# Samsung/iac

Measured on AMD Instinct MI355X. Metric: Msamples/s rendered (3rd-order HOA->binaural, 48 kHz), higher is better.
Workload: dtype f32

## Files before the change

### iac_amd/__init__.py

```python
from .hipabi import (
    FMT_F32,
    FMT_S16,
    FMT_S24,
    FMT_S32,
    KIND_DMX,
    KIND_FIR,
    KIND_H2M,
    KIND_M2M,
    PROJ_AUTO,
    PROJ_EXACT,
    PROJ_MFMA,
    SS,
    Batch,
    BatchConfig,
    DemixConfig,
    DemixFrame,
    DemixState,
    DmxFrame,
    DmxState,
    FANOUT_MAX,
    RenderArgs,
    Resampler,
    dmx_matrix,
    fir_matrix,
    IamfHipError,
    LpcmLayout,
    LpcmInput,
    Matrix,
    build,
    get_h2m_matrix,
    get_m2m_matrix,
    layout_channels,
    lib,
    lib_path,
    lpcm_unpack,
    render_fanout,
    ROUTE,
    RouteRow,
    route_instances,
    route_reset,
    route_tally,
)
```

### iac_amd/csrc/iamf_render.hip

```cpp
#include <hip/hip_runtime.h>

#include <math.h>
#include <stdint.h>
#include <atomic>
#include <stdio.h>
#include <stdlib.h>
#include <string.h>

#include <new>
#include <type_traits>
#include <vector>

#include "../../include/iamf_hip.h"

#define IAMF_FFT_HOST_TABLES

#include "render_entry.hpp"

namespace {

#include "render_common.hpp"
#include "render_downmix.hpp"
#include "render_fir.hpp"
#include "render_fir16.hpp"
// ... 72 lines not shown
  static Tables t(false), t_tv(true);
  return tv ? t_tv : t;
}

int find_matrix(int kind, int in_id, int out_id, iamf_hip_matrix *out, bool tv = false) {
  const Tables &t = tables(tv);
  if (!t.ok || !out) return -1;
  for (int i = 0; i < t.n; ++i) {
    const TableEntry &e = t.ents[i];
    if ((int)e.kind == kind && (int)e.in_id == in_id && (int)e.out_id == out_id) {
      out->kind = kind;
      out->in_id = in_id;
      out->out_id = out_id;
      out->channels = e.channels;
      out->lfe1 = e.lfe1;
      out->lfe2 = e.lfe2;
      out->m = e.m;
      out->n = e.n;
      out->mat = t.data + e.offset;
      return 0;
    }
  }
  return -1;
}

float ease(float x) {
  if (1.0 < x) return 1.0f;
  if (x < 0) return 0.0f;
  return 1.0f - powf(x - 1, 2.0);
}

}

struct iamf_hip_batch {
  iamf_hip_batch_config cfg;
  int device = 0;
  hipEvent_t done = nullptr;
  bool rendered = false;
  int m = 0, n_feeds = 0;
  int32_t src_feed[kMaxOut];
  uint32_t nz_mask[6] = {0, 0, 0, 0, 0, 0};
  int sparse = 0;
  int32_t *d_src_feed = nullptr;
  float thr = 0.f;
  int n_atk = 0, n_end = 0;
  std::vector<int64_t> spos;
  std::vector<uint8_t> sflushed;
  bool any_rendered = false;
  bool lp_scale_ok = false;
  float *d_matrix = nullptr, *d_gains = nullptr, *d_ctab = nullptr, *d_ring_y = nullptr,
        *d_ring_pm = nullptr;
  LimState *d_lim = nullptr;
  std::vector<float> h_gains;
  bool has2 = false;
  int m2 = 0;
  float *d_matrix2 = nullptr, *d_gains2 = nullptr;
  int32_t *d_src_feed2 = nullptr, *d_dmx_tab = nullptr;
  bool dmx = false;
  int dmx_n_in = 0, dmx_n_out = 0;
  float *d_pre = nullptr;
  int pre_l = 0;
  std::vector<float> h_fm;
  float *d_matrix_pre = nullptr;
  uint32_t nz_mask_pre[6] = {0, 0, 0, 0, 0, 0};
  int sparse_pre = 0;
  bool demix = false;
  int demix_steps = 0, demix_skip = 0, demix_layout = 0, demix_gmask = 0, demix_w4 = 0;
  int32_t *d_demix_tab = nullptr;
  float *d_demix_ftab = nullptr;
  bool fir = false;
  int fir_taps = 0;
  float *d_fir_hist[2] = {nullptr, nullptr};
  void *d_fir_h16 = nullptr;
  float *d_fir_pq = nullptr, *d_fir_tw = nullptr;
  float *d_fir_zero = nullptr;
  float *d_fir_pre[2] = {nullptr, nullptr};
  size_t fir_pre_bytes = 0;
  float *d_fir_y = nullptr;
  size_t fir_y_floats = 0;
  float *d_lp_in = nullptr;
  size_t lp_in_floats = 0;
  float *d_fir_id = nullptr;
  int32_t *d_fir_id_feed = nullptr;
  float fir_inv_scale = 1.f;
  int fir_cur = 0;
  bool lfe = false;
  float lfe_a1 = 0.f, lfe_a2 = 0.f, lfe_a3 = 0.f, lfe_b1 = 0.f, lfe_b2 = 0.f;
  double lfe_div = 0.0;
  float *d_lfe_state = nullptr, *d_lfe_next = nullptr, *d_lfe_u = nullptr;
  bool lfe_shared = false;
  size_t lfe_u_floats = 0;
  uint8_t *d_nat = nullptr;
  size_t nat_bytes = 0;
  uint8_t *d_dump = nullptr;
};

namespace {

bool on_batch_device(const iamf_hip_batch *b) {
  int dev = -1;
  return hipGetDevice(&dev) == hipSuccess && dev == b->device;
}

int quiesce(iamf_hip_batch *b) {
  if (b->rendered) HIPCHK(hipEventSynchronize(b->done));
  return IAMF_HIP_OK;
// ... 521 lines not shown
    b->dmx_n_out = mx.n;
    for (int i = 0; i < mx.m; ++i) dmx_tab[i] = kLayoutCh[mx.in_id][i];
    for (int i = 0; i < mx.n; ++i) dmx_tab[12 + i] = kLayoutCh[mx.out_id][i];
  } else if (fir) {
    for (int i = 0; i < kMaxOut; ++i) b->src_feed[i] = -1;
    fm.assign(mx.mat, mx.mat + (size_t)2 * mx.m * cfg->fir_taps);
  } else {
    build_feed_map(mx, cfg->out_channels, fm, b->src_feed);
    b->lp_scale_ok = true;
    for (float w : fm)
      if (w != 0.f && !(fabsf(w) >= 0x1p-100f && fabsf(w) <= 0x1p100f)) b->lp_scale_ok = false;
    if (cfg->lfe_hoa && mx.kind == IAMF_HIP_KIND_H2M && (mx.lfe1 >= 0 || mx.lfe2 >= 0)) {
      const float sample_rate = (float)cfg->sample_rate, cutoff_freq = 120;
      const float delta_time = 1 / sample_rate + 1.0e-10;
      const float c = 1.0f / (float)tanf(M_PI * cutoff_freq * delta_time);
      b->lfe = true;
      b->lfe_a1 = 1.0f / (1.0f + c + c * c);
      b->lfe_a2 = 2.0f * b->lfe_a1;
      b->lfe_a3 = b->lfe_a1;
      b->lfe_b1 = 2.0f * (1.0f - c * c) * b->lfe_a1;
      b->lfe_b2 = (1.0f - c + c * c) * b->lfe_a1;
      b->lfe_div = mx.n <= 2 ? 0.0 : sqrt((double)mx.n);
      if (mx.lfe1 >= 0 && mx.lfe1 < cfg->out_channels) b->src_feed[mx.lfe1] = -2;
      if (mx.lfe2 >= 0 && mx.lfe2 < cfg->out_channels) b->src_feed[mx.lfe2] = -2;
    }
    int set = 0, all = 0;
    for (int g = 0; g < 6 && 4 * g < cfg->out_channels; ++g)
      for (int k = 0; k < mx.m && k < 32; ++k) {
        bool nz = false;
        for (int c = 4 * g; c < 4 * g + 4 && c < cfg->out_channels; ++c)
          if (b->src_feed[c] >= 0 && fm[(size_t)b->src_feed[c] * mx.m + k] != 0.f) nz = true;
        ++all;
        if (nz) {
          ++set;
          b->nz_mask[g] |= 1u << k;
        }
      }
    b->sparse = 2 * set < all ? 1 : 0;
    b->h_fm = fm;
  }

  const float atk = 0.001f, rel = 0.200f;
  b->thr = (float)pow(10, cfg->limiter_threshold_db / 20);
  const float inc = (float)1 / (float)cfg->sample_rate;
  std::vector<float> T;
  T.push_back(0.0f);
  while (T.back() < rel + atk && T.size() < (1u << 22)) T.push_back(T.back() + inc);
  b->n_end = (int)T.size() - 1;
  b->n_atk = 0;
  while (b->n_atk < b->n_end && T[b->n_atk] < atk) ++b->n_atk;
  std::vector<float> ctab((size_t)b->n_end + 1, 1.0f);
  for (int k = 1; k <= b->n_end; ++k)
    ctab[k] = (k - 1) < b->n_atk ? ease(T[k] / atk) : ease((T[k] - atk) / rel);

  const int ns = cfg->n_streams;
  b->h_gains.assign((size_t)3 * ns, 1.0f);
#define CREATE_CHK(expr)                       \
  do {                                         \
    if ((expr) != hipSuccess) {                \
      iamf_hip_batch_destroy(b);               \
      return IAMF_HIP_ERR_DEVICE;              \
    }                                          \
  } while (0)
  CREATE_CHK(hipEventCreateWithFlags(&b->done, hipEventDisableTiming));
  CREATE_CHK(hipMalloc(&b->d_matrix, sizeof(float) * fm.size()));
  CREATE_CHK(hipMalloc(&b->d_gains, sizeof(float) * 3 * ns));
  CREATE_CHK(hipMalloc(&b->d_ctab, sizeof(float) * ctab.size()));
  CREATE_CHK(hipMalloc(&b->d_lim, sizeof(LimState) * ns));
  CREATE_CHK(hipMalloc(&b->d_ring_y, sizeof(float) * (size_t)ns * cfg->out_channels * kSave));
  CREATE_CHK(hipMalloc(&b->d_ring_pm, sizeof(float) * (size_t)ns * kSave));
  if (b->lfe) {
    CREATE_CHK(hipMalloc(&b->d_lfe_state, sizeof(float) * 4 * (size_t)ns));
    CREATE_CHK(hipMalloc(&b->d_lfe_next, sizeof(float) * 2 * (size_t)ns));
  }
  CREATE_CHK(hipMalloc(&b->d_dump, (size_t)ns * 256 * 16));
  CREATE_CHK(hipMalloc(&b->d_src_feed, sizeof(int32_t) * kMaxOut));
  CREATE_CHK(hipMemcpy(b->d_src_feed, b->src_feed, sizeof(int32_t) * kMaxOut, hipMemcpyHostToDevice));
  if (fir) {
    const size_t hb = sizeof(float) * (size_t)ns * mx.m * 256;
    CREATE_CHK(hipMalloc(&b->d_fir_hist[0], hb));
    CREATE_CHK(hipMalloc(&b->d_fir_hist[1], hb));
    CREATE_CHK(hipMemset(b->d_fir_hist[0], 0, hb));
    CREATE_CHK(hipMemset(b->d_fir_hist[1], 0, hb));
    const int taps = cfg->fir_taps;
    float hmax = 0.f;
    for (size_t i = 0; i < (size_t)2 * mx.m * taps; ++i) hmax = fmaxf(hmax, fabsf(mx.mat[i]));
    if (hmax > 0.f && hmax < 1e30f) {
      int e = 0;
      (void)frexpf(hmax, &e);
      const float scale = ldexpf(1.f, 14 - e);
      std::vector<_Float16> tab((size_t)mx.m * 2 * 2 * 8 * kF16Taps, (_Float16)0.f);
      for (int ch = 0; ch < mx.m; ++ch)
        for (int ear = 0; ear < 2; ++ear)
          for (int r = 0; r < 8; ++r)
            for (int n = 0; n < kF16Taps; ++n) {
              const int k = n + r - 15;
              if (k < 0 || k >= taps) continue;
              const float v = mx.mat[((size_t)ear * mx.m + ch) * taps + k] * scale;
              const _Float16 hi = (_Float16)v;
              const _Float16 lo = (_Float16)((v - (float)hi) * 2048.f);
              const size_t at = ((((size_t)ch * 2 + ear) * 2 + 0) * 8 + r) * kF16Taps + n;
              tab[at] = hi;
              tab[at + (size_t)8 * kF16Taps] = lo;
            }
      CREATE_CHK(hipMalloc(&b->d_fir_h16, tab.size() * sizeof(_Float16)));
      CREATE_CHK(hipMemcpy(b->d_fir_h16, tab.data(), tab.size() * sizeof(_Float16), hipMemcpyHostToDevice));
// ... 196 lines not shown
  hipStream_t st = static_cast<hipStream_t>(args->stream);
  const size_t need = (size_t)ns * nf * ch * fs;
  if (need > b->lp_in_floats) {
    const int q = quiesce(b);
    if (q != IAMF_HIP_OK) return q;
    HIPCHK(hipStreamSynchronize(st));
    (void)hipFree(b->d_lp_in);
    b->d_lp_in = nullptr;
    b->lp_in_floats = 0;
    HIPCHK(hipMalloc(&b->d_lp_in, sizeof(float) * need));
    HIPCHK(hipMemset(b->d_lp_in, 0, sizeof(float) * need));
    b->lp_in_floats = need;
  }
  const int fmax = 65535 / n_streams > 0 ? 65535 / n_streams : 0;
  if (fmax == 0) return IAMF_HIP_ERR_UNIMPLEMENTED;
  const int64_t lp_stream_stride = (int64_t)nf * ch * fs;
  for (int f = 0; f < nf; f += fmax) {
    const int r = iamf_hip_lpcm_unpack_frames(
        &L, static_cast<const uint8_t *>(in->d_raw) + (int64_t)stream0 * in->raw_stream_stride + (int64_t)f * in->raw_frame_stride,
        in->raw_stream_stride, in->raw_frame_stride, nf - f < fmax ? nf - f : fmax, nullptr, 0,
        b->d_lp_in + (int64_t)stream0 * lp_stream_stride + (size_t)f * ch * fs, lp_stream_stride, (int64_t)ch * fs, n_streams, st, first,
        count);
    if (r != IAMF_HIP_OK) return r;
  }
  a.d_in = b->d_lp_in;
  a.in_stream_stride = lp_stream_stride;
  a.in_frame_stride = (int64_t)ch * fs;
  return render_range_impl(b, &a, stream0, n_streams, nullptr);
}

int iamf_hip_batch_render_ex(iamf_hip_batch *b, const iamf_hip_render_args *a) {
  if (!b) return IAMF_HIP_ERR_BAD_ARG;
  return iamf_hip_batch_render_range(b, a, 0, b->cfg.n_streams);
}

int iamf_hip_batch_render(iamf_hip_batch *b, const float *d_in, int64_t in_stream_stride,
                          int64_t in_frame_stride, int32_t n_frames, void *d_pcm,
                          int64_t pcm_stream_stride_bytes, void *stream) {
  iamf_hip_render_args a;
  memset(&a, 0, sizeof(a));
  a.d_in = d_in;
  a.in_stream_stride = in_stream_stride;
  a.in_frame_stride = in_frame_stride;
  a.n_frames = n_frames;
  a.d_pcm = d_pcm;
  a.pcm_stream_stride_bytes = pcm_stream_stride_bytes;
  a.stream = stream;
  if (b && (b->has2 || b->dmx || b->demix)) return IAMF_HIP_ERR_BAD_ARG;
  return iamf_hip_batch_render_ex(b, &a);
}

static const int kFanFuseMax = IAMF_HIP_FANOUT_MAX;

int iamf_hip_batch_render_fanout(iamf_hip_batch *const *batches, int32_t n_batches, const float *d_in, int64_t in_stream_stride,
                                 int64_t in_frame_stride, int32_t n_frames, void *const *d_pcm,
                                 const int64_t *pcm_stream_stride_bytes, void *stream, int32_t *n_emitted, int32_t *n_fused) {
  if (n_batches < 1 || n_batches > IAMF_HIP_FANOUT_MAX) return IAMF_HIP_ERR_BAD_ARG;
  if (!batches || !d_in || !d_pcm || !pcm_stream_stride_bytes || !n_emitted) return IAMF_HIP_ERR_BAD_ARG;
  for (int j = 0; j < n_batches; ++j) {
    if (!batches[j] || !d_pcm[j]) return IAMF_HIP_ERR_BAD_ARG;
    for (int i = 0; i < j; ++i)
      if (batches[i] == batches[j]) return IAMF_HIP_ERR_BAD_ARG;
  }
  iamf_hip_render_args args[IAMF_HIP_FANOUT_MAX];
  int64_t total = 0;
  const iamf_hip_batch *b0 = batches[0];
  for (int j = 0; j < n_batches; ++j) {
    const iamf_hip_batch *b = batches[j];
    if (b->cfg.n_streams != b0->cfg.n_streams || b->cfg.frame_size != b0->cfg.frame_size || b->m != b0->m ||
        (b->d_pre ? b->pre_l : b->m) != (b0->d_pre ? b0->pre_l : b0->m))
      return IAMF_HIP_ERR_BAD_ARG;
    if (b->has2 || b->dmx || b->demix) return IAMF_HIP_ERR_BAD_ARG;
    iamf_hip_render_args &a = args[j];
    memset(&a, 0, sizeof(a));
    a.d_in = d_in;
    a.in_stream_stride = in_stream_stride;
    a.in_frame_stride = in_frame_stride;
    a.n_frames = n_frames;
    a.d_pcm = d_pcm[j];
    a.pcm_stream_stride_bytes = pcm_stream_stride_bytes[j];
    a.stream = stream;
    int64_t tj = 0;
    const int rc = range_args_check(b, &a, 0, b->cfg.n_streams, &tj);
    if (rc != IAMF_HIP_OK) return rc;
    total = tj;
  }
  if (total == 0) {
    if (n_fused) *n_fused = 0;
    for (int j = 0; j < n_batches; ++j) n_emitted[j] = 0;
    return IAMF_HIP_OK;
  }
  for (int j = 0; j < n_batches; ++j) {
    const iamf_hip_batch *b = batches[j];
    if (!on_batch_device(b)) return IAMF_HIP_ERR_INVALID_STATE;
    for (int i = 0; i < b->cfg.n_streams; ++i)
      if (b->spos[(size_t)i] != b0->spos[0] || b->sflushed[(size_t)i]) return IAMF_HIP_ERR_INVALID_STATE;
  }
  if (n_fused) *n_fused = 0;
  for (int j = 0; j < n_batches; ++j) n_emitted[j] = 0;

  const int ns = b0->cfg.n_streams;
  PreparedCall pcs[IAMF_HIP_FANOUT_MAX];
  bool fuse[IAMF_HIP_FANOUT_MAX];
  int k = 0;
  for (int j = 0; j < n_batches; ++j) {
    iamf_hip_batch *b = batches[j];
    fuse[j] = false;
    const int sc = b->cfg.pcm_stride_channels;
    if (k >= kFanFuseMax || b->fir || b->lfe || b->d_pre || (sc > 0 && sc != b->cfg.out_channels) || !b->cfg.limiter_enable ||
        b->cfg.out_channels > 2)
      continue;
    const int rc = render_prepare(b, args[j], (int)total, 0, ns, nullptr, pcs[j]);
    if (rc != IAMF_HIP_OK) return rc;
    const Route r = pick_route(pcs[j].p, pcs[j].m_eff);
    fuse[j] = r.family == Family::Fast && r.variant == 0 && pcs[j].m_eff == b0->m && FanM::has(pcs[j].m_eff);
    if (fuse[j]) ++k;
  }
  if (k < 2) k = 0;
  if (k) {
    FanParams fp;
    memset(&fp, 0, sizeof(fp));
    int n = 0;
    for (int j = 0; j < n_batches; ++j) {
      if (!fuse[j]) continue;
      const RenderParams &p = pcs[j].p;
      if (n == 0) {
        fp.in = p.in;
        fp.in_stream_stride = p.in_stream_stride;
        fp.in_frame_stride = p.in_frame_stride;
        fp.pos0 = p.pos0;
        fp.total = p.total;
        fp.frame_size = p.frame_size;
        fp.n_streams = p.n_streams;
        fp.stream0 = 0;
        fp.n_launch = ns;
      }
      FanMember &mb = fp.mem[n++];
      mb.pcm = p.pcm;
      mb.pcm_stream_stride = p.pcm_stream_stride;
      mb.matrix = p.matrix;
      mb.gains = p.gains;
      mb.ctab = p.ctab;
      mb.lim = p.lim;
      mb.ring_y = p.ring_y;
      mb.ring_pm = p.ring_pm;
      mb.src_feed = p.src_feed;
      mb.out_ch = p.out_ch;
      mb.out_format = p.out_format;
      mb.loudness_on = p.loudness_on;
      mb.n_atk = p.n_atk;
      mb.n_end = p.n_end;
      mb.thr = p.thr;
    }
    if (!iamf_hip_fanout_launch(&fp, b0->m, k, static_cast<hipStream_t>(stream))) return IAMF_HIP_ERR_INTERNAL;
    HIPCHK(hipGetLastError());
    iamf_hip_route_count(IAMF_HIP_ROUTE_FANOUT, 0, b0->m, 0, k);
    for (int j = 0; j < n_batches; ++j) {
      if (!fuse[j]) continue;
      const int r = render_commit(batches[j], pcs[j]);
      if (r < 0) return r;
      n_emitted[j] = r;
    }
    if (n_fused) *n_fused = k;
  }
  for (int j = 0; j < n_batches; ++j) {
    if (k && fuse[j]) continue;
    const int r = render_call(batches[j], args[j], (int)total, 0, ns);
    if (r < 0) return r;
    n_emitted[j] = r;
  }
  return IAMF_HIP_OK;
}

int iamf_hip_batch_flush_range(iamf_hip_batch *b, void *d_pcm, int64_t pcm_stream_stride_bytes, void *stream,
                               int32_t stream0, int32_t n_streams) {
  if (!b || !d_pcm) return IAMF_HIP_ERR_BAD_ARG;
  if (stream0 < 0 || n_streams <= 0 || stream0 + n_streams > b->cfg.n_streams) return IAMF_HIP_ERR_BAD_ARG;
  for (int i = stream0; i < stream0 + n_streams; ++i)
    if (b->sflushed[(size_t)i]) return IAMF_HIP_ERR_INVALID_STATE;
  if (!b->cfg.limiter_enable) return 0;
  iamf_hip_render_args a;
  memset(&a, 0, sizeof(a));
  a.d_pcm = d_pcm;
  a.pcm_stream_stride_bytes = pcm_stream_stride_bytes;
  a.stream = stream;
  const int r = render_call(b, a, kDelay, stream0, n_streams);
  if (r >= 0)
    for (int i = stream0; i < stream0 + n_streams; ++i) b->sflushed[(size_t)i] = 1;
  return r;
}

int iamf_hip_batch_flush(iamf_hip_batch *b, void *d_pcm, int64_t pcm_stream_stride_bytes, void *stream) {
  if (!b) return IAMF_HIP_ERR_BAD_ARG;
  return iamf_hip_batch_flush_range(b, d_pcm, pcm_stream_stride_bytes, stream, 0, b->cfg.n_streams);
}

int iamf_hip_batch_set_second_element(iamf_hip_batch *b, const iamf_hip_matrix *mx, const float *g2) {
  if (b && !on_batch_device(b)) return IAMF_HIP_ERR_INVALID_STATE;
  if (!b || !mx || !mx->mat || mx->m <= 0 || mx->m > kMaxIn || mx->n <= 0 || mx->n > kMaxOut ||
      mx->kind == IAMF_HIP_KIND_DMX || b->any_rendered)
    return IAMF_HIP_ERR_BAD_ARG;
  std::vector<float> fm;
  int32_t feed[kMaxOut];
  build_feed_map(*mx, b->cfg.out_channels, fm, feed);
  const int ns = b->cfg.n_streams;
  std::vector<float> gains((size_t)ns, 1.0f);
  if (g2) memcpy(gains.data(), g2, sizeof(float) * ns);
  (void)hipFree(b->d_matrix2);
  (void)hipFree(b->d_gains2);
// ... 298 lines not shown
```

### iac_amd/csrc/iamf_render_fanout.hip

```cpp
#include <hip/hip_runtime.h>

#include <stdint.h>
#include <atomic>
#include <stdlib.h>
#include <string.h>

#include <type_traits>

#include "../../include/iamf_hip.h"
#include "render_entry.hpp"

namespace {

#include "render_common.hpp"
#include "render_downmix.hpp"
#include "render_fir.hpp"
#include "render_fir16.hpp"
#include "render_fir_fft.hpp"
#include "render_fast.hpp"
#include "render_fanout.hpp"

static_assert(2 * sizeof(float) * fan_lds_floats(3, 16) <= 160 * 1024, "K = 2 and 3: two workgroups per CU");
static_assert(sizeof(float) * fan_lds_floats(kFanMax, 16) <= 160 * 1024, "K = 4 fits a CU");

static_assert(FanK::has(2) && FanK::has(kFanMax) && !FanK::has(kFanMax + 1), "FanK is 2..kFanMax");

template <int M, int K>
void launch_fan_mk(const FanParams &p, hipStream_t st) {
  constexpr size_t lds = sizeof(float) * (size_t)fan_lds_floats(K, M);
  launch_big_lds<&render_fanout_kernel<M, K>, (int)lds>(dim3((unsigned)p.n_launch), dim3(256), lds, st, p);
}

}

int iamf_hip_fanout_launch(const void *params, int m, int k, hipStream_t st) {
  FanParams p;
  memcpy(&p, params, sizeof(p));
  for (int j = 0; j < k && j < kFanMax; ++j)
    if (p.mem[j].out_ch < 1 || p.mem[j].out_ch > 2) return 0;
  return dispatch(FanM{}, m, [&](auto M) {
    return dispatch(FanK{}, k, [&](auto K) { launch_fan_mk<M.value, K.value>(p, st); });
  });
}
```

### iac_amd/csrc/render_fanout.hpp

```cpp
#pragma once

constexpr int kFanMax = IAMF_HIP_FANOUT_MAX;

struct FanMember {
  uint8_t *pcm;
  int64_t pcm_stream_stride;
  const float *matrix;
  const float *gains;
  const float *ctab;
  LimState *lim;
  float *ring_y;
  float *ring_pm;
  const int32_t *src_feed;
  int32_t out_ch;
  int32_t out_format;
  int32_t loudness_on;
  int32_t n_atk, n_end;
  float thr;
};

struct FanParams {
  const float *in;
  int64_t in_stream_stride;
  int64_t in_frame_stride;
  int64_t pos0;
  int32_t total;
  int32_t frame_size;
  int32_t n_streams;
  int32_t stream0, n_launch;
  FanMember mem[kFanMax];
};

__host__ __device__ constexpr int fan_member_floats() { return 3 * kFRing + 2 * (kFRing / 16) + kSave + 2 * kFWin; }
__host__ __device__ constexpr int fan_lds_floats(int k, int m) {
  return k * fan_member_floats() + kFChunk + ((2 * k * m + 15) & ~15) + 16;
}

template <int M, int K>
__global__ __launch_bounds__(256, K <= 3 ? 2 : 1) void render_fanout_kernel(const FanParams p) {
  static_assert(K >= 2 && K <= kFanMax, "two to four members");
  extern __shared__ float lds[];
  constexpr int R = kFRing;
  constexpr int NB = R / 16;
  constexpr int MB = fan_member_floats();
  constexpr int NS = 2 * K;
  constexpr int oSuf = 2 * R, oBm = 3 * R, oPm = 3 * R + 2 * NB, oWin = oPm + kSave, oHead = oWin + kFWin;
  float *arr_p = lds + K * MB;
  float *arr_g = arr_p;
  float *mat = arr_p + kFChunk;
  float *misc = mat + ((NS * M + 15) & ~15);
  constexpr bool kWG = (M % 4) == 0;

  const int s = blockIdx.x + p.stream0;
  const int t = (int)threadIdx.x;
  const int wave = t >> 6;
  const int lane = t & 63;
  const int q = t & 3;
  const int fs = p.frame_size;
  int base = (int)((p.pos0 & ~(int64_t)15) % R);

  float g_cur[K], gs[K], ge[K], m_eg[K], m_og[K], m_lg[K];
  int n_st[K];
  bool any_gain[K], live[K][2];
#pragma unroll
  for (int j = 0; j < K; ++j) {
    const FanMember &mb = p.mem[j];
    float *my = lds + j * MB;
    const int oc = mb.out_ch;
    const float *sy = mb.ring_y + (int64_t)s * oc * kSave;
    const float *spm = mb.ring_pm + (int64_t)s * kSave;
    const int rp = ring_wrap(base - kSave + t);
#pragma unroll
    for (int c = 0; c < 2; ++c)
      if (c < oc) my[c * R + rp] = sy[c * kSave + t];
    const float pm = spm[t];
    my[oPm + t] = pm;
    float sfx = pm;
    sfx = fmaxf(sfx, __shfl_down(sfx, 1, 16));
    sfx = fmaxf(sfx, __shfl_down(sfx, 2, 16));
    sfx = fmaxf(sfx, __shfl_down(sfx, 4, 16));
    sfx = fmaxf(sfx, __shfl_down(sfx, 8, 16));
    my[oSuf + rp] = sfx;
    if ((t & 15) == 0) my[oBm + (rp >> 4)] = my[oBm + (rp >> 4) + NB] = sfx;
    const int n_end = mb.n_end;
    for (int i = t; i < kFWin; i += 256) my[oHead + i] = mb.ctab[i < n_end ? i : n_end];
    if (t < 2 * M) {
      const int c = t / M, m = t - c * M;
      const int f = c < oc ? mb.src_feed[c] : -1;
      mat[2 * j * M + t] = f >= 0 ? mb.matrix[f * M + m] : 0.f;
    }
    const LimState ls = mb.lim[s];
    g_cur[j] = ls.g, gs[j] = ls.gs, ge[j] = ls.ge, n_st[j] = ls.n;
    const float eg = mb.gains[s], og = mb.gains[p.n_streams + s], lg = mb.gains[2 * p.n_streams + s];
    const bool eg_on = (eg != 1.f && eg > 0.f);
    const bool og_on = (og != 1.f && og > 0.f);
    const bool lg_on = mb.loudness_on && (lg != 1.0f);
    m_eg[j] = eg_on ? eg : 1.f, m_og[j] = og_on ? og : 1.f, m_lg[j] = lg_on ? lg : 1.f;
    any_gain[j] = eg_on || og_on || lg_on;
#pragma unroll
    for (int c = 0; c < 2; ++c) live[j][c] = c < oc && mb.src_feed[c] >= 0;
  }
  chain_wave_publish(misc + 12);

  const int64_t out_base = p.pos0 > kDelay ? p.pos0 - kDelay : 0;
  const float *in_s = p.in + (int64_t)s * p.in_stream_stride;

  float4 x[M];
  const __amdgpu_buffer_rsrc_t rs_in =
      __builtin_amdgcn_make_buffer_rsrc(const_cast<void *>(static_cast<const void *>(in_s)), 0, 0x7fffffff, 0x00020000);
  const __amdgpu_buffer_rsrc_t rs_none =
      __builtin_amdgcn_make_buffer_rsrc(const_cast<void *>(static_cast<const void *>(in_s)), 0, 0, 0x00020000);
  const bool fr_uni = (fs & (kFChunk - 1)) == 0;
  int fu = 0, iu = 0;
  auto frame_pos = [&](int kq, int &f, int &i) {
    if (fr_uni) {
      f = fu;
      i = iu + 4 * t;
    } else {
      f = kq / fs;
      i = kq - f * fs;
    }
  };
  auto load_one = [&](int m, int f, int i, __amdgpu_buffer_rsrc_t rs) {
    const int vo = 4 * (f * (int)p.in_frame_stride + i);
    const auto v = __builtin_amdgcn_raw_buffer_load_b128(rs, vo, 4 * m * fs, 2 );
    x[m] = make_float4(__uint_as_float(v[0]), __uint_as_float(v[1]), __uint_as_float(v[2]), __uint_as_float(v[3]));
  };
  {
    const int k = 4 * t;
    if (k < p.total) {
      int f, i;
      frame_pos(k, f, i);
#pragma unroll
      for (int m = 0; m < M; ++m) load_one(m, f, i, rs_in);
    } else {
#pragma unroll
      for (int m = 0; m < M; ++m) x[m] = make_float4(0.f, 0.f, 0.f, 0.f);
    }
  }
  __syncthreads();
  const int cw = chain_wave_pick(misc + 12);

  float wv[K][5];
  auto fetch_window = [&](int j, int n0) {
    const FanMember &mb = p.mem[j];
#pragma unroll
    for (int r = 0; r < 5; ++r) {
      const int i = n0 + 1 + t + 256 * r;
      wv[j][r] = 1.0f;
      if (n0 < mb.n_end && t + 256 * r < kFWin) wv[j][r] = mb.ctab[i < mb.n_end ? i : mb.n_end];
    }
  };
#pragma unroll
  for (int j = 0; j < K; ++j) fetch_window(j, n_st[j]);

  for (int c0 = 0; c0 < p.total; c0 += kFChunk) {
    const int cnt = p.total - c0 < kFChunk ? p.total - c0 : kFChunk;
    const int k = c0 + 4 * t;
    const bool valid = 4 * t < cnt;
    const int64_t gk = p.pos0 + k;
    const int rp = ring_wrap(base + 4 * t);
    const int rd = ring_wrap(base + 4 * t - kDelay);
    const int nblk = cnt >> 6;

#pragma unroll
    for (int j = 0; j < K; ++j)
#pragma unroll
      for (int r = 0; r < 5; ++r)
        if (t + 256 * r < kFWin) lds[j * MB + oWin + t + 256 * r] = wv[j][r];
    int pf_f = 0, pf_i = 0;
    __amdgpu_buffer_rsrc_t rs_pf = rs_none;
    {
      const int kn = k + kFChunk;
      iu += kFChunk;
      if (iu >= fs) {
        iu -= fs;
        ++fu;
      }
      if (c0 + kFChunk < p.total) rs_pf = rs_in;
      frame_pos(kn, pf_f, pf_i);
      if (kn >= p.total) pf_f = pf_i = 0;
    }

    using f2 = __attribute__((ext_vector_type(2))) float;
    f2 prj[2 * NS];
#pragma unroll
    for (int c = 0; c < 2 * NS; ++c) prj[c] = f2{0.f, 0.f};
    {
      float wg[NS][4];
#pragma unroll
      for (int m = 0; m < M; ++m) {
        if constexpr (kWG) {
          if ((m & 3) == 0) {
#pragma unroll
            for (int c = 0; c < NS; ++c) {
              const float4 w4 = *reinterpret_cast<const float4 *>(&mat[c * M + m]);
              wg[c][0] = w4.x, wg[c][1] = w4.y, wg[c][2] = w4.z, wg[c][3] = w4.w;
            }
          }
        }
#pragma unroll
        for (int c = 0; c < 2 * NS; ++c) asm volatile("" : "+v"(prj[c]));
        asm volatile("" : "+v"(x[m].x), "+v"(x[m].y), "+v"(x[m].z), "+v"(x[m].w));
        const f2 xa = f2{x[m].x, x[m].y};
        const f2 xb = f2{x[m].z, x[m].w};
#pragma unroll
        for (int c = 0; c < NS; ++c) {
          const float w = kWG ? wg[c][m & 3] : mat[c * M + m];
          const f2 w2 = {w, w};
          prj[2 * c] = prj[2 * c] + w2 * xa;
          prj[2 * c + 1] = prj[2 * c + 1] + w2 * xb;
        }
        load_one(m, pf_f, pf_i, rs_pf);
      }
    }

#pragma unroll
    for (int j = 0; j < K; ++j) {
      const FanMember &mb = p.mem[j];
      float *ring_y = lds + j * MB;
      float *pm_tail = ring_y + oPm;
      float *ring_suf = ring_y + oSuf;
      float *ring_bm = ring_y + oBm;
      const float *win = ring_y + oWin;
      const float *head = ring_y + oHead;
      const int oc = mb.out_ch;
      const float thr = mb.thr;
      const int n_atk = mb.n_atk, n_end = mb.n_end;

      float4 y[2];
      float4 pm = make_float4(0.f, 0.f, 0.f, 0.f);
#pragma unroll
      for (int c = 0; c < 2; ++c) {
        float4 v = make_float4(0.f, 0.f, 0.f, 0.f);
        if (live[j][c]) v = make_float4(prj[2 * (2 * j + c)].x, prj[2 * (2 * j + c)].y, prj[2 * (2 * j + c) + 1].x, prj[2 * (2 * j + c) + 1].y);
        if (any_gain[j]) {
          v.x = ((v.x * m_eg[j]) * m_og[j]) * m_lg[j];
          v.y = ((v.y * m_eg[j]) * m_og[j]) * m_lg[j];
          v.z = ((v.z * m_eg[j]) * m_og[j]) * m_lg[j];
          v.w = ((v.w * m_eg[j]) * m_og[j]) * m_lg[j];
        }
        y[c] = v;
        pm.x = fmaxf(pm.x, fabsf(v.x));
        pm.y = fmaxf(pm.y, fabsf(v.y));
        pm.z = fmaxf(pm.z, fabsf(v.z));
        pm.w = fmaxf(pm.w, fabsf(v.w));
      }

      float4 pre_ex;
      {
        const float i0 = pm.x, i1 = fmaxf(i0, pm.y), i2 = fmaxf(i1, pm.z), i3 = fmaxf(i2, pm.w);
        const float s3 = pm.w, s2 = fmaxf(pm.z, s3), s1 = fmaxf(pm.y, s2), s0 = fmaxf(pm.x, s1);
        const float qa = dpp_quad_bcast0(i3), qb = dpp_quad_bcast1(i3), qc = dpp_quad_bcast2(i3), qd = dpp_quad_bcast3(i3);
        const float before = fmaxf(fmaxf(q >= 1 ? qa : 0.f, q >= 2 ? qb : 0.f), q >= 3 ? qc : 0.f);
        const float after = fmaxf(fmaxf(q <= 2 ? qd : 0.f, q <= 1 ? qc : 0.f), q <= 0 ? qb : 0.f);
        pre_ex = make_float4(before, fmaxf(before, i0), fmaxf(before, i1), fmaxf(before, i2));
        if (valid) {
#pragma unroll
          for (int c = 0; c < 2; ++c) *reinterpret_cast<float4 *>(&ring_y[c * R + rp]) = y[c];
          if (4 * t >= cnt - kSave) *reinterpret_cast<float4 *>(&pm_tail[(c0 + 4 * t) & (kSave - 1)]) = pm;
          *reinterpret_cast<float4 *>(&ring_suf[rp]) =
              make_float4(fmaxf(s0, after), fmaxf(s1, after), fmaxf(s2, after), fmaxf(s3, after));
          if (q == 0) ring_bm[rp >> 4] = ring_bm[(rp >> 4) + NB] = fmaxf(fmaxf(qa, qb), fmaxf(qc, qd));
        }
      }
      __syncthreads();

      float4 g = make_float4(1.f, 1.f, 1.f, 1.f);
      float4 pk4;
      {
        const float *bm = ring_bm + ((rp >> 4) + NB - 14 + (q < 3 ? 4 * q : 10));
        float w14 = fmaxf(fmaxf(bm[0], bm[1]), fmaxf(bm[2], bm[3]));
        w14 = fmaxf(w14, __int_as_float(__builtin_amdgcn_update_dpp(0, __float_as_int(w14), 0xB1, 0xf, 0xf, true)));
        w14 = fmaxf(w14, __int_as_float(__builtin_amdgcn_update_dpp(0, __float_as_int(w14), 0x4E, 0xf, 0xf, true)));
        const float4 so = *reinterpret_cast<const float4 *>(&ring_suf[rd]);
        pk4.x = fmaxf(fmaxf(so.x, w14), pre_ex.x);
        pk4.y = fmaxf(fmaxf(so.y, w14), pre_ex.y);
        pk4.z = fmaxf(fmaxf(so.z, w14), pre_ex.z);
        pk4.w = fmaxf(fmaxf(so.w, w14), pre_ex.w);
        *reinterpret_cast<float4 *>(&arr_p[4 * t]) = pk4;
      }
// ... 182 lines not shown
```

### iac_amd/hipabi.py

```python
import ctypes as C
import os
import subprocess

ROOT = os.path.dirname(os.path.dirname(os.path.abspath(__file__)))
CSRC = os.path.join(ROOT, "iac_amd", "csrc")

FMT_S16, FMT_S24, FMT_S32, FMT_F32 = 16, 24, 32, -32
KIND_H2M, KIND_M2M, KIND_DMX, KIND_FIR = 0, 1, 2, 3
PROJ_AUTO, PROJ_EXACT, PROJ_MFMA = 0, 1, 2
SS = dict(A=0x020, B=0x050, C=0x250, D=0x450, E=0x451, F=0x370, G=0x490, H=0x9A3, I=0x070,
          J=0x470, STEREO=0x200, L51=0x510, L512=0x512, L514=0x514, L71=0x710, L714=0x714,
          MONO=0x100, L712=0x712, L312=0x312, BINAURAL=0x1020)

FP = C.POINTER(C.c_float)


class IamfHipError(RuntimeError):
    def __init__(self, code, what):
        super().__init__("%s failed with IAMF_HIP error %d" % (what, code))
        self.code = code


class Matrix(C.Structure):
    _fields_ = [("kind", C.c_int32), ("in_id", C.c_int32), ("out_id", C.c_int32),
# ... 57 lines not shown

class DemixState(C.Structure):
    _fields_ = [("mode", C.c_int32), ("last_mode", C.c_int32), ("w_idx", C.c_int32), ("last_w_idx", C.c_int32),
                ("last_sfavg", C.c_float * 24)]


class DemixFrame(C.Structure):
    _fields_ = [("prev", C.c_float * 5), ("cur", C.c_float * 5), ("n_recon", C.c_int32),
                ("recon_ch", C.c_int32 * 12), ("recon_prev", C.c_float * 12), ("recon_cur", C.c_float * 12)]


def lib_path():
    return os.environ.get("IAMF_HIP_LIB") or os.path.join(ROOT, "iac_amd", "lib", "libiamf_hip.so")


def build(force=False):
    args = ["make", "-j4", "-C", CSRC]
    if force:
        subprocess.check_call(args + ["clean"], stdout=subprocess.DEVNULL)
    subprocess.check_call(args, stdout=subprocess.DEVNULL)
    return lib_path()


_lib = None


def lib():
    global _lib
    if _lib is None:
        path = lib_path()
        if not os.path.exists(path):
            raise ImportError("libiamf_hip.so is not built (run __graft_entry__.build()); "
                              "iac_amd has no CPU fallback")
        L = C.CDLL(path)
        L.iamf_hip_get_h2m_matrix.argtypes = [C.c_int, C.c_int, C.POINTER(Matrix)]
        L.iamf_hip_get_m2m_matrix.argtypes = [C.c_int, C.c_int, C.POINTER(Matrix)]
        L.iamf_hip_probe_traffic.argtypes = [C.c_int, C.c_int, C.c_int, C.c_int, C.c_void_p, C.c_int64, C.c_void_p,
                                             C.c_int64, C.c_void_p]
        L.iamf_hip_pick_buffer_pair.argtypes = [C.c_int, C.c_int, C.c_int, C.c_int, C.POINTER(C.c_void_p), C.c_int, C.c_int64,
                                                C.POINTER(C.c_void_p), C.c_int, C.c_int64, C.c_void_p,
                                                C.POINTER(C.c_int), C.POINTER(C.c_int), FP]
        L.iamf_hip_get_m2m_matrix_variant.argtypes = [C.c_int, C.c_int, C.c_int, C.POINTER(Matrix)]
        L.iamf_hip_layout_channels.argtypes = [C.c_int]
        L.iamf_hip_batch_create.argtypes = [C.POINTER(BatchConfig), C.POINTER(C.c_void_p)]
        L.iamf_hip_batch_destroy.argtypes = [C.c_void_p]
        L.iamf_hip_batch_destroy.restype = None
        L.iamf_hip_batch_set_gains.argtypes = [C.c_void_p, FP, FP, FP]
        L.iamf_hip_batch_render.argtypes = [C.c_void_p, C.c_void_p, C.c_int64, C.c_int64, C.c_int32,
                                            C.c_void_p, C.c_int64, C.c_void_p]
        L.iamf_hip_batch_flush.argtypes = [C.c_void_p, C.c_void_p, C.c_int64, C.c_void_p]
        L.iamf_hip_batch_render_fanout.argtypes = [C.POINTER(C.c_void_p), C.c_int32, C.c_void_p, C.c_int64, C.c_int64, C.c_int32,
                                                   C.POINTER(C.c_void_p), C.POINTER(C.c_int64), C.c_void_p,
                                                   C.POINTER(C.c_int32), C.POINTER(C.c_int32)]
        L.iamf_hip_batch_reset.argtypes = [C.c_void_p]
        L.iamf_hip_batch_render_range.argtypes = [C.c_void_p, C.POINTER(RenderArgs), C.c_int32, C.c_int32]
        L.iamf_hip_batch_flush_range.argtypes = [C.c_void_p, C.c_void_p, C.c_int64, C.c_void_p, C.c_int32, C.c_int32]
        L.iamf_hip_format_bytes.argtypes = [C.c_int]
        L.iamf_hip_version.restype = C.c_char_p
        L.iamf_hip_batch_render_ex.argtypes = [C.c_void_p, C.POINTER(RenderArgs)]
        L.iamf_hip_batch_render_lpcm.argtypes = [C.c_void_p, C.POINTER(LpcmInput), C.POINTER(RenderArgs)]
        L.iamf_hip_batch_set_second_element.argtypes = [C.c_void_p, C.POINTER(Matrix), FP]
        L.iamf_hip_resampler_create.argtypes = [C.c_int, C.c_int, C.c_int, C.c_int, C.POINTER(C.c_void_p)]
        L.iamf_hip_resampler_destroy.argtypes = [C.c_void_p]
        L.iamf_hip_resampler_destroy.restype = None
        L.iamf_hip_resampler_out_capacity.argtypes = [C.c_void_p, C.c_int]
        L.iamf_hip_resampler_flush_capacity.argtypes = [C.c_void_p]
        L.iamf_hip_resampler_process.argtypes = [C.c_void_p, C.c_void_p, C.c_int64, C.c_int, C.c_void_p, C.c_int64,
                                                 C.c_void_p]
        L.iamf_hip_resampler_flush.argtypes = [C.c_void_p, C.c_void_p, C.c_int64, C.c_void_p]
        L.iamf_hip_resampler_process_range.argtypes = [C.c_void_p, C.c_void_p, C.c_int64, C.c_int, C.c_void_p, C.c_int64,
                                                       C.c_void_p, C.c_int32, C.c_int32]
        L.iamf_hip_resampler_flush_range.argtypes = [C.c_void_p, C.c_void_p, C.c_int64, C.c_void_p, C.c_int32, C.c_int32]
        L.iamf_hip_resampler_same_state.argtypes = [C.c_void_p, C.c_int32, C.c_int32]
        L.iamf_hip_stream_signal.argtypes = [C.c_void_p, C.c_void_p, C.c_uint32]
        L.iamf_hip_deinterleave_f32.argtypes = [C.c_void_p, C.c_int64, C.c_int32, C.c_int32, C.c_int32, C.c_void_p, C.c_int64,
                                                C.c_int64, C.c_void_p]
        L.iamf_hip_batch_set_projection.argtypes = [C.c_void_p, FP, C.c_int]
        L.iamf_hip_batch_share_lfe_state.argtypes = [C.c_void_p, C.c_void_p]
        L.iamf_hip_batch_lfe_advance.argtypes = [C.c_void_p, C.c_void_p, C.c_int64, C.c_int32, C.c_void_p, C.c_int32, C.c_int32]
        L.iamf_hip_lpcm_unpack.argtypes = [C.POINTER(LpcmLayout), C.c_void_p, C.c_int64, C.c_void_p, C.c_int64, C.c_void_p,
                                           C.c_int64, C.c_int32, C.c_void_p]
        L.iamf_hip_batch_set_demixer.argtypes = [C.c_void_p, C.POINTER(DemixConfig)]
        L.iamf_hip_demix_state_init.argtypes = [C.POINTER(DemixState)]
        L.iamf_hip_demix_state_init.restype = None
        L.iamf_hip_demix_set_info.argtypes = [C.POINTER(DemixState), C.c_int, C.c_int]
        L.iamf_hip_demix_frame_fill.argtypes = [C.POINTER(DemixState), C.c_int, C.POINTER(C.c_int32), FP,
                                                C.POINTER(DemixFrame)]
        L.iamf_hip_demix_frame_fill.restype = None
        L.iamf_hip_dmx_valid.argtypes = [C.c_int, C.c_int]
        L.iamf_hip_dmx_layout_channels.argtypes = [C.c_int]
        L.iamf_hip_dmx_state_init.argtypes = [C.POINTER(DmxState)]
        L.iamf_hip_dmx_state_init.restype = None
        L.iamf_hip_dmx_set_mode_weight.argtypes = [C.POINTER(DmxState), C.c_int, C.c_int]
        L.iamf_hip_dmx_coefficients.argtypes = [C.POINTER(DmxState), FP]
        L.iamf_hip_dmx_coefficients.restype = None
        L.iamf_hip_route_instances.argtypes = [C.POINTER(RouteRow), C.c_int]
        L.iamf_hip_route_tally.argtypes = [C.POINTER(RouteRow), C.c_int, C.c_int]
        L.iamf_hip_shard_split.argtypes = [C.c_int, C.c_int, C.c_int, C.POINTER(C.c_int), C.POINTER(C.c_int)]
        L.iamf_hip_shard_create.argtypes = [C.POINTER(BatchConfig), C.POINTER(C.c_int), C.c_int, C.POINTER(C.c_void_p)]
        L.iamf_hip_shard_destroy.argtypes = [C.c_void_p]
        L.iamf_hip_shard_destroy.restype = None
        L.iamf_hip_shard_devices.argtypes = [C.c_void_p]
        L.iamf_hip_shard_info.argtypes = [C.c_void_p, C.c_int, C.POINTER(C.c_int), C.POINTER(C.c_int), C.POINTER(C.c_int)]
        L.iamf_hip_shard_batch.argtypes = [C.c_void_p, C.c_int]
        L.iamf_hip_shard_batch.restype = C.c_void_p
        L.iamf_hip_shard_render_stream.argtypes = [C.c_void_p, C.c_int]
# ... 43 lines not shown
    m.mat = h.ctypes.data_as(FP)
    m._keep = h
    return m


def lpcm_unpack(layout, d_raw, raw_stream_stride, d_first_count, d_out, out_stream_stride, n_streams, stream=None,
                first_count_stride=2):
    r = lib().iamf_hip_lpcm_unpack(C.byref(layout), d_raw, raw_stream_stride, d_first_count, first_count_stride, d_out,
                                   out_stream_stride, n_streams, stream)
    if r < 0:
        raise IamfHipError(r, "iamf_hip_lpcm_unpack")
    return r


def route_instances():
    L = lib()
    n = L.iamf_hip_route_instances(None, 0)
    rows = (RouteRow * max(n, 1))()
    n = min(n, L.iamf_hip_route_instances(rows, n))
    return [(ROUTE_NAME[r.family], r.variant, r.m, r.c, r.k) for r in rows[:n]]


def route_tally(reset=True):
    L = lib()
    cap = L.iamf_hip_route_instances(None, 0) + 1
    rows = (RouteRow * cap)()
    n = L.iamf_hip_route_tally(rows, cap, 1 if reset else 0)
    return {(ROUTE_NAME[r.family], r.variant, r.m, r.c, r.k): r.launches for r in rows[:min(n, cap)]}


def route_reset():
    lib().iamf_hip_route_tally(None, 0, 1)


FANOUT_MAX = 4


def render_fanout(batches, d_in, in_stream_stride, in_frame_stride, n_frames, d_pcms, pcm_strides, stream=None):
    n = len(batches)
    if len(d_pcms) != n or len(pcm_strides) != n:
        raise ValueError("render_fanout: one PCM buffer and one stride per batch")
    hs = (C.c_void_p * n)(*[b.h for b in batches])
    pcms = (C.c_void_p * n)(*d_pcms)
    strides = (C.c_int64 * n)(*pcm_strides)
    emitted = (C.c_int32 * max(n, 1))()
    fused = C.c_int32(0)
    r = lib().iamf_hip_batch_render_fanout(hs, n, d_in, in_stream_stride, in_frame_stride, n_frames, pcms, strides, stream,
                                           emitted, C.byref(fused))
    if r < 0:
        raise IamfHipError(r, "iamf_hip_batch_render_fanout")
    return list(emitted[:n]), fused.value


def layout_channels(out_id):
    return lib().iamf_hip_layout_channels(out_id)


def _fparr(a):
    if a is None:
        return None
    arr = (C.c_float * len(a))(*[float(v) for v in a])
    return arr


class Batch:

    def __init__(self, n_streams, matrix, out_channels, frame_size=1024, sample_rate=48000,
                 out_format=FMT_S16, limiter=True, threshold_db=-1.0, loudness=False, projection=PROJ_AUTO, fir_taps=0,
                 lfe_hoa=False, pcm_stride_channels=0):
        cfg = BatchConfig()
        cfg.n_streams = n_streams
        cfg.frame_size = frame_size
        cfg.sample_rate = sample_rate
        cfg.out_channels = out_channels
        cfg.out_format = out_format
        cfg.matrix = matrix
        cfg.limiter_enable = 1 if limiter else 0
        cfg.limiter_threshold_db = threshold_db
        cfg.loudness_enable = 1 if loudness else 0
        cfg.projection = projection
        cfg.fir_taps = fir_taps
        cfg.lfe_hoa = 1 if lfe_hoa else 0
        cfg.pcm_stride_channels = pcm_stride_channels
        self.cfg = cfg
        self.bytes_per_sample = lib().iamf_hip_format_bytes(out_format)
        h = C.c_void_p()
        r = lib().iamf_hip_batch_create(C.byref(cfg), C.byref(h))
        if r != 0:
            raise IamfHipError(r, "iamf_hip_batch_create")
        self.h = h

    def set_gains(self, element=None, output=None, loudness=None):
        r = lib().iamf_hip_batch_set_gains(self.h, _fparr(element), _fparr(output), _fparr(loudness))
        if r != 0:
            raise IamfHipError(r, "iamf_hip_batch_set_gains")

    def render(self, d_in, in_stream_stride, in_frame_stride, n_frames, d_pcm, pcm_stream_stride_bytes,
               stream=None):
        r = lib().iamf_hip_batch_render(self.h, d_in, in_stream_stride, in_frame_stride, n_frames,
                                        d_pcm, pcm_stream_stride_bytes, stream)
        if r < 0:
            raise IamfHipError(r, "iamf_hip_batch_render")
        return r

    def render_ex(self, args):
        r = lib().iamf_hip_batch_render_ex(self.h, C.byref(args))
# ... 125 lines not shown
```

### include/iamf_hip.h

```cpp
#ifndef IAMF_HIP_H
#define IAMF_HIP_H

#include <stddef.h>
#include <stdint.h>

#ifdef __cplusplus
extern "C" {
#endif

enum {
  IAMF_HIP_OK = 0,
  IAMF_HIP_ERR_BAD_ARG = -1,
  IAMF_HIP_ERR_BUFFER_TOO_SMALL = -2,
  IAMF_HIP_ERR_INTERNAL = -3,
  IAMF_HIP_ERR_INVALID_STATE = -5,
  IAMF_HIP_ERR_UNIMPLEMENTED = -6,
  IAMF_HIP_ERR_ALLOC_FAIL = -7,
  IAMF_HIP_ERR_DEVICE = -100
};

enum {
  IAMF_HIP_SS_A = 0x020, IAMF_HIP_SS_B = 0x050, IAMF_HIP_SS_C = 0x250, IAMF_HIP_SS_D = 0x450,
  IAMF_HIP_SS_E = 0x451, IAMF_HIP_SS_F = 0x370, IAMF_HIP_SS_G = 0x490, IAMF_HIP_SS_H = 0x9A3,
  IAMF_HIP_SS_I = 0x070, IAMF_HIP_SS_J = 0x470,
// ... 94 lines not shown
} iamf_hip_demix_config;

int iamf_hip_batch_set_demixer(iamf_hip_batch *b, const iamf_hip_demix_config *cfg);

typedef struct iamf_hip_demix_state {
  int32_t mode, last_mode, w_idx, last_w_idx;
  float last_sfavg[24];
} iamf_hip_demix_state;

typedef struct iamf_hip_demix_frame {
  float prev[5], cur[5];
  int32_t n_recon;
  int32_t recon_ch[12];
  float recon_prev[12], recon_cur[12];
} iamf_hip_demix_frame;

void iamf_hip_demix_state_init(iamf_hip_demix_state *st);
int iamf_hip_demix_set_info(iamf_hip_demix_state *st, int mode, int w_idx);
void iamf_hip_demix_frame_fill(iamf_hip_demix_state *st, int n_recon, const int32_t *recon_ch,
                               const float *recon_gain, iamf_hip_demix_frame *out);

typedef struct {
  const float *d_in;
  int64_t in_stream_stride, in_frame_stride;
  const float *d_in2;
  int64_t in2_stream_stride, in2_frame_stride;
  const float *d_element_ramp, *d_element2_ramp, *d_output_ramp;
  int64_t ramp_stream_stride;
  const iamf_hip_dmx_frame *d_dmx_frames;
  int32_t n_frames;
  int32_t n_samples;
  void *d_pcm;
  int64_t pcm_stream_stride_bytes;
  void *stream;
  const iamf_hip_demix_frame *d_demix_frames;
  int32_t demix_sample0;
  int32_t lfe_pre_samples, lfe_post_samples, reserved0;
} iamf_hip_render_args;

int iamf_hip_batch_render_ex(iamf_hip_batch *b, const iamf_hip_render_args *args);

int iamf_hip_batch_render_range(iamf_hip_batch *b, const iamf_hip_render_args *args, int32_t stream0, int32_t n_streams);
int iamf_hip_batch_flush_range(iamf_hip_batch *b, void *d_pcm, int64_t pcm_stream_stride_bytes, void *stream,
                               int32_t stream0, int32_t n_streams);

int iamf_hip_batch_flush(iamf_hip_batch *b, void *d_pcm, int64_t pcm_stream_stride_bytes,
                         void *stream);

#define IAMF_HIP_FANOUT_MAX 4
int iamf_hip_batch_render_fanout(iamf_hip_batch *const *batches, int32_t n_batches, const float *d_in,
                                 int64_t in_stream_stride, int64_t in_frame_stride, int32_t n_frames, void *const *d_pcm,
                                 const int64_t *pcm_stream_stride_bytes, void *stream, int32_t *n_emitted ,
                                 int32_t *n_fused );

typedef struct iamf_hip_resampler iamf_hip_resampler;
int iamf_hip_resampler_create(int n_streams, int channels, int in_rate, int out_rate,
                              iamf_hip_resampler **out);
void iamf_hip_resampler_destroy(iamf_hip_resampler *r);
int iamf_hip_resampler_out_capacity(const iamf_hip_resampler *r, int ns);
int iamf_hip_resampler_flush_capacity(const iamf_hip_resampler *r);
int iamf_hip_resampler_process(iamf_hip_resampler *r, const float *d_in, int64_t in_stream_stride,
                               int ns, float *d_out, int64_t out_stream_stride, void *stream);
int iamf_hip_resampler_flush(iamf_hip_resampler *r, float *d_out, int64_t out_stream_stride, void *stream);
int iamf_hip_resampler_process_range(iamf_hip_resampler *r, const float *d_in, int64_t in_stream_stride, int ns, float *d_out,
                                     int64_t out_stream_stride, void *stream, int32_t stream0, int32_t n_streams);
int iamf_hip_resampler_flush_range(iamf_hip_resampler *r, float *d_out, int64_t out_stream_stride, void *stream, int32_t stream0,
                                   int32_t n_streams);
int iamf_hip_resampler_same_state(const iamf_hip_resampler *r, int32_t stream_a, int32_t stream_b);

int iamf_hip_batch_reset(iamf_hip_batch *b);

int iamf_hip_format_bytes(int out_format);
const char *iamf_hip_version(void);

int iamf_hip_probe_traffic(int n_streams, int chunks, int rows, int pieces, const void *d_in,
                           int64_t in_stream_stride_bytes, void *d_out, int64_t out_stream_stride_bytes,
                           void *stream);
int iamf_hip_pick_buffer_pair(int n_streams, int chunks, int rows, int pieces, const void *const *d_in_candidates,
                              int n_in, int64_t in_stream_stride_bytes, void *const *d_out_candidates, int n_out,
                              int64_t out_stream_stride_bytes, void *stream, int *best_in, int *best_out, float *ms);

int iamf_hip_selftest_shared_divisor(float divisor, uint64_t counts[3]);

int iamf_hip_decoder_set_hoa_lfe(void *decoder_handle, int enable);
int iamf_hip_decoder_set_variant(void *decoder_handle, int variant);

typedef struct iamf_hip_shard iamf_hip_shard;
int iamf_hip_shard_split(int n_streams, int n_devices, int index, int *first, int *count);
int iamf_hip_shard_create(const iamf_hip_batch_config *cfg, const int *devices, int n_devices, iamf_hip_shard **out);
void iamf_hip_shard_destroy(iamf_hip_shard *s);
int iamf_hip_shard_devices(const iamf_hip_shard *s);
int iamf_hip_shard_info(const iamf_hip_shard *s, int index, int *device, int *first, int *count);
iamf_hip_batch *iamf_hip_shard_batch(iamf_hip_shard *s, int index);
void *iamf_hip_shard_render_stream(iamf_hip_shard *s, int index);
int iamf_hip_shard_render(iamf_hip_shard *s, const float *const *d_in, int64_t in_stream_stride, int64_t in_frame_stride,
                          int32_t n_frames, void *const *d_pcm, int64_t pcm_stream_stride_bytes);
int iamf_hip_shard_flush(iamf_hip_shard *s, void *const *d_pcm, int64_t pcm_stream_stride_bytes);
int iamf_hip_shard_gather(iamf_hip_shard *s, int root_index, void *d_dst, int64_t dst_stream_stride_bytes,
                          void *const *d_pcm, int64_t pcm_stream_stride_bytes);
int iamf_hip_shard_gather_rows(iamf_hip_shard *s, int root_index, void *d_dst, int64_t dst_stream_stride_bytes,
                               void *const *d_pcm, int64_t pcm_stream_stride_bytes, int64_t bytes_per_stream);
int iamf_hip_shard_sync(iamf_hip_shard *s);
int iamf_hip_shard_times(iamf_hip_shard *s, int index, int64_t *last_sent_bytes, int64_t *total_sent_bytes,
                         int64_t *last_received_bytes, double *last_gather_ms, double *total_gather_ms);
const char *iamf_hip_shard_rccl_version(void);

// ... 75 lines not shown
```

Baseline: 87000.

## Share limiter window tables across K=4 fanout members to fit two workgroups per CU

When four batches fuse into one fanout launch and their limiter curve tables match, the per-member window and head tables are stored once in LDS instead of four times. This cuts the K=4 LDS footprint enough for two workgroups per CU, and launch bounds are raised to 2 for every K. A host-side memcmp decides whether the tables can be shared, and a counter of shared launches is exposed for inspection. The catch is that launch bounds of 2 at K=4 may push registers toward spilling, and the window table is now rewritten inside the per-member loop.

```diff
diff --git a/iac_amd/__init__.py b/iac_amd/__init__.py
--- a/iac_amd/__init__.py
+++ b/iac_amd/__init__.py
@@ -22,6 +22,7 @@
     RenderArgs,
     Resampler,
     dmx_matrix,
+    fanout_shared_launches,
     fir_matrix,
     IamfHipError,
     LpcmLayout,
diff --git a/iac_amd/csrc/iamf_render.hip b/iac_amd/csrc/iamf_render.hip
--- a/iac_amd/csrc/iamf_render.hip
+++ b/iac_amd/csrc/iamf_render.hip
@@ -148,6 +148,7 @@
         *d_ring_pm = nullptr;
   LimState *d_lim = nullptr;
   std::vector<float> h_gains;
+  std::vector<float> h_ctab;
   bool has2 = false;
   int m2 = 0;
   float *d_matrix2 = nullptr, *d_gains2 = nullptr;
@@ -775,6 +776,7 @@
   std::vector<float> ctab((size_t)b->n_end + 1, 1.0f);
   for (int k = 1; k <= b->n_end; ++k)
     ctab[k] = (k - 1) < b->n_atk ? ease(T[k] / atk) : ease((T[k] - atk) / rel);
+  b->h_ctab = ctab;
 
   const int ns = cfg->n_streams;
   b->h_gains.assign((size_t)3 * ns, 1.0f);
@@ -1077,6 +1079,12 @@
 
 static const int kFanFuseMax = IAMF_HIP_FANOUT_MAX;
 
+static std::atomic<int64_t> g_fan_shared_launches;
+
+int64_t iamf_hip_fanout_shared_launches(int reset) {
+  return reset ? g_fan_shared_launches.exchange(0, std::memory_order_relaxed) : g_fan_shared_launches.load(std::memory_order_relaxed);
+}
+
 int iamf_hip_batch_render_fanout(iamf_hip_batch *const *batches, int32_t n_batches, const float *d_in, int64_t in_stream_stride,
                                  int64_t in_frame_stride, int32_t n_frames, void *const *d_pcm,
                                  const int64_t *pcm_stream_stride_bytes, void *stream, int32_t *n_emitted, int32_t *n_fused) {
@@ -1146,8 +1154,15 @@
     FanParams fp;
     memset(&fp, 0, sizeof(fp));
     int n = 0;
+    const iamf_hip_batch *first = nullptr;
+    fp.tab_shared = k == kFanSplit;
     for (int j = 0; j < n_batches; ++j) {
       if (!fuse[j]) continue;
+      const iamf_hip_batch *b = batches[j];
+      if (!first) first = b;
+      else if (fp.tab_shared && (b->n_atk != first->n_atk || b->n_end != first->n_end ||
+                                 memcmp(b->h_ctab.data(), first->h_ctab.data(), sizeof(float) * b->h_ctab.size()) != 0))
+        fp.tab_shared = 0;
       const RenderParams &p = pcs[j].p;
       if (n == 0) {
         fp.in = p.in;
@@ -1180,6 +1195,7 @@
     if (!iamf_hip_fanout_launch(&fp, b0->m, k, static_cast<hipStream_t>(stream))) return IAMF_HIP_ERR_INTERNAL;
     HIPCHK(hipGetLastError());
     iamf_hip_route_count(IAMF_HIP_ROUTE_FANOUT, 0, b0->m, 0, k);
+    if (fp.tab_shared) g_fan_shared_launches.fetch_add(1, std::memory_order_relaxed);
     for (int j = 0; j < n_batches; ++j) {
       if (!fuse[j]) continue;
       const int r = render_commit(batches[j], pcs[j]);
diff --git a/iac_amd/csrc/iamf_render_fanout.hip b/iac_amd/csrc/iamf_render_fanout.hip
--- a/iac_amd/csrc/iamf_render_fanout.hip
+++ b/iac_amd/csrc/iamf_render_fanout.hip
@@ -1,5 +1,6 @@
 #include <hip/hip_runtime.h>
 
+#include <stddef.h>
 #include <stdint.h>
 #include <atomic>
 #include <stdlib.h>
@@ -21,14 +22,17 @@
 #include "render_fanout.hpp"
 
 static_assert(2 * sizeof(float) * fan_lds_floats(3, 16) <= 160 * 1024, "K = 2 and 3: two workgroups per CU");
+static_assert(2 * sizeof(float) * fan_lds_floats(kFanMax, 16, true) <= 160 * 1024, "K = 4, equal tables: two workgroups per CU");
 static_assert(sizeof(float) * fan_lds_floats(kFanMax, 16) <= 160 * 1024, "K = 4 fits a CU");
+static_assert(offsetof(FanParams, mem) == offsetof(FanParams, tab_shared) + sizeof(int32_t), "tab_shared takes the place of padding");
 
 static_assert(FanK::has(2) && FanK::has(kFanMax) && !FanK::has(kFanMax + 1), "FanK is 2..kFanMax");
 
 template <int M, int K>
 void launch_fan_mk(const FanParams &p, hipStream_t st) {
-  constexpr size_t lds = sizeof(float) * (size_t)fan_lds_floats(K, M);
-  launch_big_lds<&render_fanout_kernel<M, K>, (int)lds>(dim3((unsigned)p.n_launch), dim3(256), lds, st, p);
+  constexpr size_t cap = sizeof(float) * (size_t)fan_lds_floats(K, M);
+  const size_t lds = sizeof(float) * (size_t)fan_lds_floats(K, M, p.tab_shared != 0);
+  launch_big_lds<&render_fanout_kernel<M, K>, (int)cap>(dim3((unsigned)p.n_launch), dim3(256), lds, st, p);
 }
 
 }
diff --git a/iac_amd/csrc/render_fanout.hpp b/iac_amd/csrc/render_fanout.hpp
--- a/iac_amd/csrc/render_fanout.hpp
+++ b/iac_amd/csrc/render_fanout.hpp
@@ -28,27 +28,33 @@
   int32_t frame_size;
   int32_t n_streams;
   int32_t stream0, n_launch;
+  int32_t tab_shared;
   FanMember mem[kFanMax];
 };
 
-__host__ __device__ constexpr int fan_member_floats() { return 3 * kFRing + 2 * (kFRing / 16) + kSave + 2 * kFWin; }
-__host__ __device__ constexpr int fan_lds_floats(int k, int m) {
-  return k * fan_member_floats() + kFChunk + ((2 * k * m + 15) & ~15) + 16;
+__host__ __device__ constexpr int fan_core_floats() { return 3 * kFRing + 2 * (kFRing / 16) + kSave; }
+__host__ __device__ constexpr int fan_member_floats() { return fan_core_floats() + 2 * kFWin; }
+constexpr int kFanSplit = 4;
+__host__ __device__ constexpr int fan_lds_floats(int k, int m, bool tab_shared = false) {
+  return k * fan_core_floats() + (k == kFanSplit && tab_shared ? 1 : k) * 2 * kFWin + kFChunk + ((2 * k * m + 15) & ~15) + 16;
 }
 
 template <int M, int K>
-__global__ __launch_bounds__(256, K <= 3 ? 2 : 1) void render_fanout_kernel(const FanParams p) {
+__global__ __launch_bounds__(256, 2) void render_fanout_kernel(const FanParams p) {
   static_assert(K >= 2 && K <= kFanMax, "two to four members");
   extern __shared__ float lds[];
   constexpr int R = kFRing;
   constexpr int NB = R / 16;
-  constexpr int MB = fan_member_floats();
+  constexpr bool kSplit = K == kFanSplit;
+  constexpr int MB = kSplit ? fan_core_floats() : fan_member_floats();
   constexpr int NS = 2 * K;
   constexpr int oSuf = 2 * R, oBm = 3 * R, oPm = 3 * R + 2 * NB, oWin = oPm + kSave, oHead = oWin + kFWin;
   float *arr_p = lds + K * MB;
   float *arr_g = arr_p;
   float *mat = arr_p + kFChunk;
   float *misc = mat + ((NS * M + 15) & ~15);
+  float *tab = misc + 16;
+  const int tstep = p.tab_shared ? 0 : 2 * kFWin;
   constexpr bool kWG = (M % 4) == 0;
 
   const int s = blockIdx.x + p.stream0;
@@ -83,7 +89,12 @@
     my[oSuf + rp] = sfx;
     if ((t & 15) == 0) my[oBm + (rp >> 4)] = my[oBm + (rp >> 4) + NB] = sfx;
     const int n_end = mb.n_end;
-    for (int i = t; i < kFWin; i += 256) my[oHead + i] = mb.ctab[i < n_end ? i : n_end];
+    if constexpr (kSplit) {
+      if (j == 0 || !p.tab_shared)
+        for (int i = t; i < kFWin; i += 256) tab[j * tstep + kFWin + i] = mb.ctab[i < n_end ? i : n_end];
+    } else {
+      for (int i = t; i < kFWin; i += 256) my[oHead + i] = mb.ctab[i < n_end ? i : n_end];
+    }
     if (t < 2 * M) {
       const int c = t / M, m = t - c * M;
       const int f = c < oc ? mb.src_feed[c] : -1;
@@ -163,11 +174,13 @@
     const int rd = ring_wrap(base + 4 * t - kDelay);
     const int nblk = cnt >> 6;
 
-#pragma unroll
-    for (int j = 0; j < K; ++j)
-#pragma unroll
-      for (int r = 0; r < 5; ++r)
-        if (t + 256 * r < kFWin) lds[j * MB + oWin + t + 256 * r] = wv[j][r];
+    if constexpr (!kSplit) {
+#pragma unroll
+      for (int j = 0; j < K; ++j)
+#pragma unroll
+        for (int r = 0; r < 5; ++r)
+          if (t + 256 * r < kFWin) lds[j * MB + oWin + t + 256 * r] = wv[j][r];
+    }
     int pf_f = 0, pf_i = 0;
     __amdgpu_buffer_rsrc_t rs_pf = rs_none;
     {
@@ -222,11 +235,17 @@
       float *pm_tail = ring_y + oPm;
       float *ring_suf = ring_y + oSuf;
       float *ring_bm = ring_y + oBm;
-      const float *win = ring_y + oWin;
-      const float *head = ring_y + oHead;
+      const float *win = kSplit ? tab + j * tstep : ring_y + oWin;
+      const float *head = kSplit ? tab + j * tstep + kFWin : ring_y + oHead;
       const int oc = mb.out_ch;
       const float thr = mb.thr;
       const int n_atk = mb.n_atk, n_end = mb.n_end;
+
+      if constexpr (kSplit) {
+#pragma unroll
+        for (int r = 0; r < 5; ++r)
+          if (t + 256 * r < kFWin) tab[j * tstep + t + 256 * r] = wv[j][r];
+      }
 
       float4 y[2];
       float4 pm = make_float4(0.f, 0.f, 0.f, 0.f);
diff --git a/iac_amd/hipabi.py b/iac_amd/hipabi.py
--- a/iac_amd/hipabi.py
+++ b/iac_amd/hipabi.py
@@ -133,6 +133,8 @@
         L.iamf_hip_batch_render_fanout.argtypes = [C.POINTER(C.c_void_p), C.c_int32, C.c_void_p, C.c_int64, C.c_int64, C.c_int32,
                                                    C.POINTER(C.c_void_p), C.POINTER(C.c_int64), C.c_void_p,
                                                    C.POINTER(C.c_int32), C.POINTER(C.c_int32)]
+        L.iamf_hip_fanout_shared_launches.argtypes = [C.c_int]
+        L.iamf_hip_fanout_shared_launches.restype = C.c_int64
         L.iamf_hip_batch_reset.argtypes = [C.c_void_p]
         L.iamf_hip_batch_render_range.argtypes = [C.c_void_p, C.POINTER(RenderArgs), C.c_int32, C.c_int32]
         L.iamf_hip_batch_flush_range.argtypes = [C.c_void_p, C.c_void_p, C.c_int64, C.c_void_p, C.c_int32, C.c_int32]
@@ -282,6 +284,10 @@
     return list(emitted[:n]), fused.value
 
 
+def fanout_shared_launches(reset=True):
+    return lib().iamf_hip_fanout_shared_launches(1 if reset else 0)
+
+
 def layout_channels(out_id):
     return lib().iamf_hip_layout_channels(out_id)
 
diff --git a/include/iamf_hip.h b/include/iamf_hip.h
--- a/include/iamf_hip.h
+++ b/include/iamf_hip.h
@@ -170,6 +170,8 @@
                                  int64_t in_stream_stride, int64_t in_frame_stride, int32_t n_frames, void *const *d_pcm,
                                  const int64_t *pcm_stream_stride_bytes, void *stream, int32_t *n_emitted ,
                                  int32_t *n_fused );
+
+int64_t iamf_hip_fanout_shared_launches(int reset);
 
 typedef struct iamf_hip_resampler iamf_hip_resampler;
 int iamf_hip_resampler_create(int n_streams, int channels, int in_rate, int out_rate,
```

New measurement: 80240. 0.922x the previous value.
